# 10XGenomics/supernova

Measured on AMD Instinct MI355X. Metric: Gk-mers/s through count+graph at k=48, 1.2B×150bp; bit-exact counts, higher is better.
Workload: dtype u64

## Files before the change

include/snk.h:

```cpp
#ifndef SNK_H_
#define SNK_H_
#include <stddef.h>
#include <stdint.h>

#ifdef __cplusplus
extern "C" {
#endif

#define SNK_OK 0
#define SNK_E_ARG (-1)
#define SNK_E_HIP (-2)
#define SNK_E_NOGPU (-3)
#define SNK_E_NOMEM (-4)
#define SNK_E_IO (-5)
#define SNK_E_UNSUPPORTED (-6)
#define SNK_E_INTERNAL (-7)

typedef struct snk_ctx snk_ctx;

typedef struct snk_params {
    uint32_t K;
    uint32_t min_qual;
    uint32_t min_freq;
    uint32_t min_bc;
// ... 26 lines not shown
    uint32_t count_tight_slots;
    uint32_t count_screen_ratio_pct;
    uint32_t target_inst;
    uint32_t bucket_fill_pct;
    uint32_t adaptive_buckets;
    uint32_t chunk_kmers;
    uint32_t minimiser_len;
    uint32_t partition_passes;
    uint32_t hot_buckets;
    uint32_t hot_min, hot_factor, hot_class_inst;
    uint32_t exchange_ranges;
    uint32_t join_ranking;
    uint32_t path_lookup;
    uint32_t unitig_bc_cut;
    uint32_t hbv_dev_min, hbv_big;
    uint32_t reserved[9];
    uint32_t last_count_kernel, last_count_limit, last_partition_passes, last_minimiser_len;
} snk_tuning;
void snk_tuning_default(snk_tuning* t);
int snk_ctx_set_tuning(snk_ctx* ctx, const snk_tuning* t, char* err, size_t errcap);
void snk_ctx_get_tuning(const snk_ctx* ctx, snk_tuning* t);
int snk_ctx_set_option(snk_ctx* ctx, const char* name, long long value, char* err, size_t errcap);
int snk_option_check(const char* name, long long value, char* err, size_t errcap);
int snk_ctx_clear_option(snk_ctx* ctx, const char* name);
int snk_ctx_get_option(const snk_ctx* ctx, const char* name, long long* value);
const char* snk_option_name(uint32_t i);
const char* snk_option_doc(uint32_t i);

typedef struct snk_synth_params {
    uint64_t seed;
    uint64_t n_reads;
// ... 416 lines not shown
```

supernova_amd/csrc/snk_count.hip:

```cpp
#include "snk_ctx.h"
#include "snk_common.h"
#include "snk_kernels.h"
#include "snk_stages.h"

namespace {

constexpr uint32_t BC_MULTI = 0xFFFFFFFEu;
constexpr uint32_t BC_IGN = 0xFFFFFFFFu;
static_assert(BC_IGN > BC_MULTI, "barcode states are merged with atomicMax");
#ifndef SNK_TIGHT_TRIES
#define SNK_TIGHT_TRIES 48
#endif
constexpr int MAX_SPLIT_LOG2 = 20;
#define SNK_COUNT_MAXSEG 32
#ifndef SNK_COUNT_THREADS
#define SNK_COUNT_THREADS 768
#endif
#ifndef SNK_SCREEN_ROUNDS
#define SNK_SCREEN_ROUNDS 6
#endif
#ifndef SNK_GSCREEN_SLOTS
#define SNK_GSCREEN_SLOTS 1024
#endif
#ifndef SNK_GSCREEN_BATCH
// ... 10 lines not shown
#endif
#define LDS_LOAD(p) __hip_atomic_load((p), __ATOMIC_RELAXED, __HIP_MEMORY_SCOPE_WORKGROUP)
__device__ __forceinline__ void lds_barrier() { asm volatile("s_waitcnt lgkmcnt(0)\n\ts_barrier" ::: "memory"); }
#ifdef SNK_COUNT_PROF
#define PROF(n) do { if (tid == 0) { const long long _t = clock64(); prof_acc[n] += (unsigned long long)(_t - prof_t); prof_t = _t; } } while (0)
#else
#define PROF(n) do {} while (0)
#endif

__device__ __forceinline__ uint32_t funnel(uint32_t hi, uint32_t lo, uint32_t sh) {
#ifdef SNK_FUNNEL_ALIGNBIT
    return sh ? __builtin_amdgcn_alignbit(hi, lo, 32u - sh) : hi;
#else
    return (uint32_t)(((((uint64_t)hi << 32) | lo) << sh) >> 32);
#endif
}

template <int K> struct lo_t { typedef uint32_t type; };
template <> struct lo_t<60> { typedef uint64_t type; };

template <int K> __device__ __forceinline__ typename lo_t<K>::type lo_pack(uint64_t lo);
template <> __device__ __forceinline__ uint32_t lo_pack<48>(uint64_t lo) { return (uint32_t)(lo >> 32); }
template <> __device__ __forceinline__ uint64_t lo_pack<60>(uint64_t lo) { return lo; }
template <int K> __device__ __forceinline__ uint64_t lo_unpack(typename lo_t<K>::type v);
template <> __device__ __forceinline__ uint64_t lo_unpack<48>(uint32_t v) { return (uint64_t)v << 32; }
template <> __device__ __forceinline__ uint64_t lo_unpack<60>(uint64_t v) { return v; }

template <int K, bool G> struct klo_t { typedef typename lo_t<K>::type type; };
template <int K> struct klo_t<K, true> { typedef uint64_t type; };
template <int K, bool G> __device__ __forceinline__ typename klo_t<K, G>::type klo_pack(uint64_t lo) {
// ... 16 lines not shown
    uint64_t* khi = reinterpret_cast<uint64_t*>(smem_raw);
    lo_type* klo = reinterpret_cast<lo_type*>(khi + SLOTS);
    uint32_t* tag = reinterpret_cast<uint32_t*>(klo + SLOTS);
    uint32_t* cnt = tag + SLOTS;
    uint32_t* bcs = cnt + SLOTS;
    uint32_t* ctxw = bcs + SLOTS;
    uint32_t* rec = ctxw + SLOTS / 4;
    uint32_t* ctl = rec + 8 * BATCH;
    uint32_t* dd = ctl + (TIGHT ? 72 : 64);
    uint32_t* wgt = dd + DD;
    uint16_t* lead = reinterpret_cast<uint16_t*>(wgt + BATCH);
    uint16_t* lpre = lead + BATCH;
    uint16_t* cidx = lpre + BATCH + 2;
    uint32_t* segi = reinterpret_cast<uint32_t*>(smem_raw + (((size_t)(reinterpret_cast<unsigned char*>(cidx + NCI) - smem_raw) + 15) & ~(size_t)15));
    uint16_t* olist = reinterpret_cast<uint16_t*>(segi + 2 * 3 * SNK_COUNT_MAXSEG);
    uint32_t* bcx = reinterpret_cast<uint32_t*>(smem_raw + (((size_t)(reinterpret_cast<unsigned char*>(olist + (TIGHT ? SLOTS - 64 : SLOTS - THREADS - 64)) - smem_raw) + 15) & ~(size_t)15));
    const bool bcset = a.bc_mode > 2;
    constexpr int SROUNDS = (SCREEN && SLOTS <= 1024) ? SNK_GSCREEN_ROUNDS : SNK_SCREEN_ROUNDS;
    static_assert(SROUNDS >= 1 && SROUNDS <= 16, "two cells per register");
    constexpr int SPW = GROUPED ? ((DD + BATCH) / 3 >= 512 ? 512 : 256) : SNK_NGSCREEN_PLANE_WORDS;
    constexpr uint32_t SCB = SPW == 1024 ? 17u : (SPW == 512 ? 18u : 19u);
    constexpr uint32_t SCAND = GROUPED ? (SLOTS <= 1024 ? 2048 : 1024) : 4096;
    uint16_t* cand = reinterpret_cast<uint16_t*>(bcx);
    uint32_t* planes = GROUPED ? dd : reinterpret_cast<uint32_t*>(cand + SCAND);
    static_assert(!SCREEN || (GROUPED && 3 * SPW <= DD + BATCH) || (!GROUPED && K == 48 && SLOTS <= 1024), "no room for the screen's bit planes");
    static_assert(THREADS >= BATCH && THREADS % 64 == 0, "the first BATCH threads own the staged records");
    const int tid = threadIdx.x;
    const int lane = tid & 63;
    const uint32_t LIMIT = TIGHT ? min(a.tight & 0xFFFFu, (uint32_t)SLOTS - 64u) : SLOTS - THREADS - 64;
    const int tight_tries = (int)(a.tight >> 16);
#ifdef SNK_COUNT_PROF
    long long prof_t = clock64();
    unsigned long long prof_acc[8] = {0, 0, 0, 0, 0, 0, 0, 0};
#endif
    auto dma_batch = [&](uint64_t base, uint64_t vend, const uint32_t* bnd, const uint32_t* seg) {
        constexpr int CH = 2 * BATCH;
        uint32_t seg_incl = 0;
        if (MULTI) {
            const uint32_t mylen = (uint32_t)lane < a.nseg ? LDS_LOAD(&seg[2 * SNK_COUNT_MAXSEG + lane]) - LDS_LOAD(&seg[lane]) : 0u;
            seg_incl = snk_wave_scan_incl(mylen);
        }
        constexpr int NR = (CH + THREADS - 1) / THREADS;
        uint32_t gx[NR];
        if (GATHER) {
#pragma unroll
// ... 33 lines not shown
            vend = ((uint64_t)LDS_LOAD(&bnd[3]) << 32) | LDS_LOAD(&bnd[2]);
        }
    };
    const uint32_t G = a.bucket_stride;
    unsigned long long rcur = a.region_cursor[blockIdx.x];
    uint32_t bucket = a.bucket0 + (blockIdx.x + G - a.bucket0 % G) % G;
    uint32_t par = 0;
    {
        uint64_t b0 = 0, e0 = 0;
        if (tid == 0) {
            if (bucket < a.NB) { b0 = a.seg_beg[bucket]; e0 = a.seg_end[bucket]; }
            ctl[4] = (uint32_t)b0; ctl[5] = (uint32_t)(b0 >> 32); ctl[6] = (uint32_t)e0; ctl[7] = (uint32_t)(e0 >> 32);
            ctl[3] = 0;
            ctl[1] = 0; ctl[2] = 0; ctl[8] = 0; ctl[9] = 0; ctl[10] = 0; ctl[11] = 0; ctl[0] = 0;
            if (TIGHT) { ctl[64] = 0; ctl[65] = 0; }
        }
        for (int s = tid; s < SLOTS; s += THREADS) tag[s] = 0;
        if (MULTI && tid < (int)a.nseg) {
            uint64_t b = 0, e = 0;
            if (bucket < a.NB) { b = a.seg_beg[(uint64_t)tid * a.seg_stride + bucket]; e = a.seg_end[(uint64_t)tid * a.seg_stride + bucket]; }
            segi[tid] = (uint32_t)b; segi[SNK_COUNT_MAXSEG + tid] = (uint32_t)(b >> 32); segi[2 * SNK_COUNT_MAXSEG + tid] = (uint32_t)e;
        }
        lds_barrier();
        uint64_t vb, ve;
        bucket_range(ctl + 4, segi, vb, ve);
        dma_batch(vb, ve, ctl + 4, segi);
    }
    bool prefetched = true;
    uint32_t q = 0, bq = 0;
    unsigned long long claims_sum = 0;
    for (; bucket < a.NB; bucket += G) {
    uint32_t sp = 1;
    bool fresh = true;
    uint32_t splits_done = 0;
    const uint32_t nbucket = bucket + G;
    bool seg_pending = true;
    const uint32_t* bcur = ctl + 4 + 8 * par;
    uint32_t* bnext = ctl + 4 + 8 * (par ^ 1u);
    const uint32_t* segc = segi + par * (3 * SNK_COUNT_MAXSEG);
    uint32_t* segn = segi + (par ^ 1u) * (3 * SNK_COUNT_MAXSEG);
    const uint32_t sseg = MULTI ? min((uint32_t)tid, a.nseg - 1u) : 0u;
    auto load_next = [&](uint64_t& nbeg, uint64_t& nend, uint64_t& nsb, uint32_t& nse) {
        nbeg = 0; nend = 0; nsb = 0; nse = 0;
        if (nbucket < a.NB) {
            nbeg = a.seg_beg[nbucket]; nend = a.seg_end[nbucket];
            if (MULTI) { nsb = a.seg_beg[(uint64_t)sseg * a.seg_stride + nbucket]; nse = (uint32_t)a.seg_end[(uint64_t)sseg * a.seg_stride + nbucket]; }
        }
    };
    auto put_down = [&](uint64_t nbeg, uint64_t nend, uint64_t nsb, uint32_t nse) {
        bnext[0] = (uint32_t)nbeg; bnext[1] = (uint32_t)(nbeg >> 32); bnext[2] = (uint32_t)nend; bnext[3] = (uint32_t)(nend >> 32);
        if (MULTI) { segn[sseg] = (uint32_t)nsb; segn[SNK_COUNT_MAXSEG + sseg] = (uint32_t)(nsb >> 32); segn[2 * SNK_COUNT_MAXSEG + sseg] = nse; }
        seg_pending = false;
    };
    uint32_t lg0 = 0, id0 = 0, real_bucket = bucket;
    if (a.vmeta) {
        const uint2 vm = a.vmeta[bucket];
        real_bucket = __builtin_amdgcn_readfirstlane(vm.x);
        lg0 = __builtin_amdgcn_readfirstlane(vm.y >> 24);
        id0 = __builtin_amdgcn_readfirstlane(vm.y & 0xFFFFFFu);
    }
    while (sp) {
// ... 17 lines not shown
            if (seg_pending) {
                uint64_t nbeg, nend, nsb; uint32_t nse;
                load_next(nbeg, nend, nsb, nse);
                put_down(nbeg, nend, nsb, nse);
            }
            lds_barrier();
        }
        PROF(1);
        {
            for (uint64_t base = vbeg; base < vend; base += BATCH) {
                if (!prefetched) dma_batch(base, vend, bcur, segc);
                prefetched = false;
                if (tid < BATCH) wgt[tid] = (SCREEN && GROUPED) ? 0u : 1u;
                if (SCREEN && !GROUPED) { for (int qq = tid; qq < 3 * SPW; qq += THREADS) planes[qq] = 0; }
                for (int q = tid; q < DD; q += THREADS) dd[q] = 0;
                asm volatile("s_waitcnt vmcnt(0)" ::: "memory");
                lds_barrier();
                PROF(2);
                if (tid == 0) { ctl[1 + (q ^ 1u)] = 0; ctl[8 + (q ^ 1u)] = 0; ctl[10 + (bq ^ 1u)] = 0; if (TIGHT) ctl[64 + (q ^ 1u)] = 0; if (SCREEN) ctl[0] = 0; }
                const bool fetch_next = seg_pending;
                uint64_t nbeg = 0, nend = 0, nsb = 0; uint32_t nse = 0;
                if (fetch_next) load_next(nbeg, nend, nsb, nse);
                uint32_t nkm = 0;
                if (tid < BATCH && base + tid < vend) {
                    const uint4 ra = *reinterpret_cast<const uint4*>(rec + 8 * tid), rb = *reinterpret_cast<const uint4*>(rec + 8 * tid + 4);
                    nkm = rb.z & 0x7Fu;
                    if (a.dbg == 5 && ((rb.z >> 7) & 3u) != 3u) nkm = 0;
                    if (!GROUPED && a.dbg != 4 && nkm) {
                        uint32_t h = (ra.x * 0x9E3779B1u) ^ snk_rotl32(ra.y * 0x85EBCA77u, 7) ^ (ra.z * 0xC2B2AE3Du) ^ snk_rotl32(ra.w * 0x27D4EB2Fu, 13)
                                   ^ (rb.x * 0x165667B1u) ^ snk_rotl32(rb.y * 0xcc9e2d51u, 19) ^ (rb.z * 0x1b873593u);
                        h ^= h >> 15; h *= 0x846ca68bu; h ^= h >> 13;
                        uint32_t s = h & (DD - 1);
                        for (;;) {
                            uint32_t v = LDS_LOAD(&dd[s]);
                            if (v == 0) {
                                v = atomicCAS(&dd[s], 0u, (uint32_t)tid + 1u);
                                if (v == 0) break;
                            }
                            const uint32_t L = v - 1u;
                            const uint4 la = *reinterpret_cast<const uint4*>(rec + 8 * L);
                            const uint32_t lb0 = rec[8 * L + 4], lb1 = rec[8 * L + 5], lb2 = rec[8 * L + 6];
                            bool same = ((la.x ^ ra.x) | (la.y ^ ra.y) | (la.z ^ ra.z) | (la.w ^ ra.w) | (lb0 ^ rb.x) | (lb1 ^ rb.y) | (lb2 ^ rb.z)) == 0;
                            if (GROUPED || bcset) same = same && LDS_LOAD(&rec[8 * L + 7]) == rb.w;
                            if (same) {
                                atomicAdd(&wgt[L], 1u);
                                const uint32_t mine = GROUPED ? 0u : rb.w;
                                if (mine >= BC_MULTI) atomicMax(&rec[8 * L + 7], mine);
                                else if (mine) {
                                    uint32_t ob = atomicCAS(&rec[8 * L + 7], 0u, mine);
                                    if (ob != 0 && ob != mine && ob < BC_MULTI) atomicMax(&rec[8 * L + 7], BC_MULTI);
                                }
                                nkm = 0;
                                break;
                            }
                            s = (s + 1) & (DD - 1);
                        }
                    }
                }
                const uint32_t sv = nkm | (nkm ? 0x10000u : 0u);
                uint32_t incl = sv;
                incl = snk_wave_scan_incl(incl);
                uint32_t woff = 0;
                if (lane == 63 && incl) woff = atomicAdd(&ctl[10 + bq], incl);
                woff = __builtin_amdgcn_readlane(woff, 63);
                if (tid < BATCH && nkm) {
                    const uint32_t ex = woff + incl - sv;
                    const uint32_t off = ex & 0xFFFFu, r = ex >> 16;
                    lead[r] = (uint16_t)tid;
                    lpre[r] = (uint16_t)(off + nkm);
                    for (uint32_t w = (off + 31u) >> 5; (w << 5) < off + nkm; ++w) cidx[w] = (uint16_t)r;
// ... 67 lines not shown
                        if (n_iter > SCAND) { screened = false; n_iter = total; }
                    }
                }
                for (uint32_t g0 = 0; g0 < n_iter; g0 += THREADS) {
                    if (TIGHT ? (LDS_LOAD(resv) >> 31) != 0u : LDS_LOAD(occ) > LIMIT) break;
                    uint32_t g = g0 + tid;
                    const bool have = g < n_iter;
                    if (SCREEN && screened && have) g = cand[g];
                    if (have) {
                        uint32_t lr = cidx[g >> 5];
                        uint32_t lend = lpre[lr];
                        while (lend <= g) lend = lpre[++lr];
                        const uint32_t i = lead[lr];
                        const uint32_t* rp = rec + 8 * i;
                        const uint32_t m6 = rp[6], w7 = rp[7];
                        const uint32_t wt = (SCREEN && GROUPED) ? 1u : wgt[i];
                        const uint32_t n_i = m6 & 0x7Fu, hasL = (m6 >> 7) & 1u, hasR = (m6 >> 8) & 1u;
                        const uint32_t j = g + n_i - lend;
                        const uint32_t bst = GROUPED ? 0u : w7;
                        const uint32_t o = hasL + j;
                        const uint32_t wi = o >> 4, sh = (2u * o) & 31u;
                        const uint32_t* wp = rp + wi;
                        const uint32_t P = wp[-1], W0 = wp[0], W1 = wp[1], W2 = wp[2], W3 = wp[3];
                        const uint32_t F0 = funnel(W0, W1, sh), F1 = funnel(W1, W2, sh), F2 = funnel(W2, W3, sh);
                        const uint32_t pb = funnel(P, W0, sh) & 3u;
                        uint32_t F3 = 0, nb;
                        if constexpr (K == 48) nb = (W3 >> (30u - sh)) & 3u;
                        else {
                            static_assert(K == 60, "K is 48 or 60");
                            const uint32_t W4 = wp[4];
                            const uint32_t f3 = funnel(W3, W4, sh);
                            nb = (f3 >> 6) & 3u;
                            F3 = f3 & 0xFFFFFF00u;
// ... 202 lines not shown
                        const uint32_t e = atomicAdd(&a.status[4], 1u);
                        if (e < a.extra_cap) a.extra[e] = make_uint4(real_bucket, (uint32_t)rbase, nvalid | (blockIdx.x << 12), (split_lg << 24) | split_id);
                    }
                }
            }
        }
        claims_sum += nocc;
        if (tid == 0 && nocc > ctl[3]) ctl[3] = nocc;
        q ^= 1u;
        PROF(7);
    }
    if (tid == 0 && splits_done) atomicAdd(&a.status[2], 1u);
    par ^= 1u;
    }
    if (tid == 0) { a.region_cursor[blockIdx.x] = rcur; atomicMax(&a.status[3], ctl[3]); atomicAdd(&a.status[5], (uint32_t)(claims_sum >> 4)); }
    asm volatile("s_waitcnt vmcnt(0)" ::: "memory");
#ifdef SNK_COUNT_PROF
    if (tid == 0) for (int q = 0; q < 8; ++q) atomicAdd(&a.prof[q], prof_acc[q]);
#endif
}

template <int K> struct cfg;
template <> struct cfg<48> { static constexpr int THREADS = SNK_COUNT_THREADS; static constexpr int SLOTS = SNK_COUNT_SLOTS; };
template <> struct cfg<60> { static constexpr int THREADS = SNK_COUNT_THREADS; static constexpr int SLOTS = SNK_COUNT_SLOTS; };

template <int K, bool G>
size_t lds_bytes(uint32_t bc_mode = 0, bool tight = false, bool screen = false) {
    const size_t S = screen ? SNK_GSCREEN_SLOTS : cfg<K>::SLOTS, B = (G && screen && S <= 1024 && K == 48) ? SNK_GSCREEN_BATCH : ((K == 48 && !G && (S >= 2048 || screen)) ? 512 : 256), DD = 2 * B, NCI = B * (K - SNK_M_MIN_OF(K) + 1) / 32 + 2;
    return S * (8 + sizeof(typename klo_t<K, G>::type) + 4 + 4 + 4) + S + 4 * (8 * B + (tight ? 72 : 64) + DD + B) + 2 * (B + B + 2 + NCI) + 16 + 2 * 4 * 3 * SNK_COUNT_MAXSEG + 2 * (tight ? S - 64 : S - cfg<K>::THREADS - 64) + 16 + (bc_mode > 2 ? S * 24 + 16 : 0) + (screen ? (G ? (S <= 1024 ? 4096 : 2048) : 8192 + 3 * SNK_NGSCREEN_PLANE_WORDS * 4) + 16 : 0);
}

template <int K, bool G>
int launch(hipStream_t st, const snk_count_args& a, char* err, size_t errcap) {
    auto kern = a.nseg > 1 ? snk_count_kernel<K, cfg<K>::THREADS, cfg<K>::SLOTS, G, true> : snk_count_kernel<K, cfg<K>::THREADS, cfg<K>::SLOTS, G, false>;
    if (a.gidx) {
        if (a.nseg != 1) return snk_fail(SNK_E_INTERNAL, err, errcap, "count: an index list comes with one segment per bucket");
        kern = snk_count_kernel<K, cfg<K>::THREADS, cfg<K>::SLOTS, G, false, true>;
    }
    const bool tight = a.tight && !a.gidx;
    const bool screen = K == 48 && tight && a.screen >= 2u && a.bc_mode <= 2u;
    static_assert(SNK_GSCREEN_SLOTS <= 1024, "the ungrouped SCREEN instantiation needs the LDS half a table frees");
    if constexpr (K == 48) {
        if (screen) kern = a.nseg > 1 ? snk_count_kernel<K, cfg<K>::THREADS, SNK_GSCREEN_SLOTS, G, true, false, true, true> : snk_count_kernel<K, cfg<K>::THREADS, SNK_GSCREEN_SLOTS, G, false, false, true, true>;
    }
// ... 79 lines not shown
```

supernova_amd/csrc/snk_ctx.h:

```cpp
#pragma once
#include <hip/hip_runtime.h>
#include <stdarg.h>
#include <stdio.h>
#include <string.h>

#include <string>
#include <vector>

#include "../../include/snk.h"
#include "snk_launch.h"
#include "snk_opts.h"
#include "snk_plan.h"

struct snk_ctx {
    int device = 0;
    hipStream_t stream = nullptr;
    hipStream_t cur_stream = nullptr;
    int n_cu = 256;
    size_t lds_per_block = 65536;
    uint64_t device_mem_total = 0;
    double pass_sigma = 0.0;
    uint64_t plan_mapped = 0;
    uint64_t plan_mem = 0;
    struct block { void* p; size_t bytes; bool used; uint64_t serial = 0; uint64_t epoch = 0; };
// ... 18 lines not shown
    size_t cached_bytes = 0;
    uint64_t last_n_kmers = 0, last_n_instances = 0;
    uint64_t last_region_max = 0, last_region_n = 0;
    uint64_t last_bnd = 0, last_bnd_n = 0;
    uint32_t last_ovf = 0, last_ovf_nb = 0;
    uint64_t last_ovf_reads = 0;
    uint64_t last_dense = 0;
    uint32_t count_screen = 0;
    uint32_t count_tight = 0;
    snk_sizing_history sizing;
    uint32_t mlen = 16;
    uint32_t last_extra = 0;
    uint64_t last_input_fp = 0;
    bool have_input_fp = false;
    uint32_t last_count_limit = 0;
    uint32_t last_partition_passes = 1;
    std::vector<unsigned long long> h_region_off;
    snk_opts opts;
    void* shard = nullptr;
    void* host_io = nullptr;
    void (*host_io_free)(void*) = nullptr;
    void* df_io = nullptr;
    void (*df_io_free)(void*) = nullptr;
    void* stream_job = nullptr;
    void (*stream_job_free)(void*) = nullptr;
    void (*stream_job_invalidate)(void*) = nullptr;
    void* shard_host = nullptr;
    void (*shard_host_free)(void*) = nullptr;
};

// ... 25 lines not shown
```

supernova_amd/csrc/snk_opts.hip:

```cpp
#include <stdio.h>
#include <stdlib.h>
#include <string.h>

#include <string>

#include "snk_opts.h"
#ifndef SNK_OPTS_NO_CTX
#include "snk_ctx.h"
#endif

const snk_opt_def snk_opt_defs[SNK_OPT_COUNT] = {
#define X(name, dflt, range, doc) {#name, dflt, range, doc},
    SNK_OPTIONS(X)
#undef X
};

int snk_opt_index(const char* name) {
    if (!name) return -1;
    for (int i = 0; i < SNK_OPT_COUNT; ++i) if (strcmp(snk_opt_defs[i].name, name) == 0) return i;
    return -1;
}
void snk_opts_init(snk_opts* o) { memset(o, 0, sizeof *o); }

int snk_opts_parse(snk_opts* o, const char* text, char* bad, unsigned badcap) {
// ... 135 lines not shown
    long long v;
    for (const tfield& f : tfields) if (get(f.opt, &v)) *reinterpret_cast<uint32_t*>(reinterpret_cast<char*>(t) + f.off) = (uint32_t)v;
    long long tight = 0, ng = 0;
    const bool ts = get(SNK_OPT_count_tight, &tight), ns = get(SNK_OPT_count_screen_ng, &ng);
    if (ns && ng >= 2) t->count_kernel = SNK_COUNT_KERNEL_SCREEN;
    else if (ts && tight) { t->count_kernel = SNK_COUNT_KERNEL_BOOKED; t->count_tight_slots = (uint32_t)tight; }
    else if (ts) t->count_kernel = SNK_COUNT_KERNEL_MARGIN;
    if (get(SNK_OPT_adaptive_buckets, &v)) t->adaptive_buckets = v ? 1 : 2;
    if (get(SNK_OPT_hot, &v)) t->hot_buckets = v ? 1 : 2;
    if (get(SNK_OPT_path_index, &v)) t->path_lookup = v ? 1 : 2;
    if (get(SNK_OPT_join_replicated, &v)) t->join_ranking = v ? 2 : 1;
    t->last_count_limit = ctx->last_count_limit;
    t->last_count_kernel = ctx->count_screen ? SNK_COUNT_KERNEL_SCREEN : (ctx->count_tight ? SNK_COUNT_KERNEL_BOOKED : SNK_COUNT_KERNEL_MARGIN);
    t->last_partition_passes = ctx->last_partition_passes;
    t->last_minimiser_len = ctx->mlen;
}
#endif
```

supernova_amd/csrc/snk_stages.hip:

```cpp
#include <string.h>
#include <cstring>
#include <rocprim/rocprim.hpp>

#include <stdlib.h>
#include <math.h>

#include <cmath>
#include <vector>

#include "snk_ctx.h"
#include "snk_common.h"
#include "snk_graph.h"
#include "snk_kernels.h"
#include "snk_stages.h"


int snk_stage_count_table(snk_ctx* ctx, hipStream_t st, uint32_t K, const void* records, const uint64_t* seg_beg,
                          const uint64_t* seg_end, uint32_t seg_stride, uint32_t nseg, uint32_t NB, uint32_t min_freq, uint32_t bc_mode, uint32_t grouped, uint64_t n_inst_hint,
                          uint32_t* status, bool want_sort, snk_table* out, char* err, size_t errcap, const snk_count_ranges* ranges, snk_count_pilot* pilot,
                          const uint32_t* gidx, bool defer_compact, const snk_hot* hot) {
    if (hot && hot->NBv == 0) hot = nullptr;
    defer_compact = defer_compact && !want_sort && snk_opt_u32(ctx, SNK_OPT_defer_compact) != 0;
    int rc;
    snk_phase_timer tm(st), kt(st);
    tm.mark();
    uint32_t n_regions = 1;
    if ((rc = snk_count_regions(K, grouped, nseg, NB, bc_mode, snk_opt_u32(ctx, SNK_OPT_count_persist), &n_regions, err, errcap))) return rc;
    uint64_t est = n_inst_hint / (min_freq > 1 ? 12 : 1) + 4096;
    const bool tight = ranges && ranges->n > 1 && ranges->replay && min_freq > 1 && ctx->plan_mem && (double)est * 24.0 > 0.10 * (double)ctx->plan_mem;
    if (tight) est = n_inst_hint / 32 + 4096;
    if (ctx->last_n_kmers && ctx->last_n_instances == n_inst_hint) est = ctx->last_n_kmers + ctx->last_n_kmers / (tight ? 8 : 2) + 4096;
    bool range0_probe = tight && !(ctx->last_n_kmers && ctx->last_n_instances == n_inst_hint);
    uint64_t region_cap = est / n_regions + 64;
    if (ctx->last_n_kmers && ctx->last_n_instances == n_inst_hint && ctx->last_region_n == n_regions && ctx->last_region_max + ctx->last_region_max / 4 + 64 > region_cap)
        region_cap = ctx->last_region_max + ctx->last_region_max / 4 + 64;
    snk_u128 *keys_r = nullptr, *keys_a = nullptr, *keys_b = nullptr;
    uint64_t *vals_r = nullptr, *vals_a = nullptr, *vals_b = nullptr;
    unsigned long long *rcur = nullptr, *roff = nullptr;
    uint64_t n_kmers = 0;
    uint32_t h_status[8] = {0, 0, 0, 0, 0, 0, 0, 0};
    {
        void* q;
        if ((rc = snk_ctx_alloc(ctx, (n_regions + 1) * 8ull, &q, err, errcap))) return rc; rcur = (unsigned long long*)q;
        if ((rc = snk_ctx_alloc(ctx, (n_regions + 1) * 8ull, &q, err, errcap))) return rc; roff = (unsigned long long*)q;
    }
    std::vector<unsigned long long> h_rcur(n_regions);
    uint32_t *chunk_n = nullptr, *chunk_base = nullptr;
    uint4* extra = nullptr;
    uint32_t extra_cap = 0;
    if (!want_sort) {
        void* q;
        if ((rc = snk_ctx_alloc(ctx, (NB + 1) * 4ull, &q, err, errcap))) return rc; chunk_n = (uint32_t*)q;
        if ((rc = snk_ctx_alloc(ctx, (NB + 1) * 4ull, &q, err, errcap))) return rc; chunk_base = (uint32_t*)q;
        extra_cap = NB / 8 > (1u << 16) ? NB / 8 : (1u << 16);
        if (ctx->last_extra > extra_cap) extra_cap = ctx->last_extra + ctx->last_extra / 4;
        if (hot) extra_cap += hot->NBv + hot->NBv / 2;
        if (ranges && ranges->hots) extra_cap += NB / 16 + (1u << 16);
    }
    bool pilot_regrown = false;
    for (int attempt = 0; attempt < 4; ++attempt) {
        void* q;
        if (!want_sort) {
            if ((rc = snk_ctx_alloc(ctx, (size_t)extra_cap * 16 + 16, &q, err, errcap))) return rc; extra = (uint4*)q;
            SNK_HIP_TRY(hipMemsetAsync(chunk_n, 0, (NB + 1) * 4ull, st));
        }
        if ((rc = snk_ctx_alloc(ctx, region_cap * n_regions * 16, &q, err, errcap))) return rc; keys_r = (snk_u128*)q;
        if ((rc = snk_ctx_alloc(ctx, region_cap * n_regions * 8, &q, err, errcap))) return rc; vals_r = (uint64_t*)q;
        SNK_HIP_TRY(hipMemsetAsync(rcur, 0, (n_regions + 1) * 8ull, st));
        SNK_HIP_TRY(hipMemsetAsync(status, 0, 32, st));
        snk_count_args ca;
        ca.records = (const uint4*)records;
        ca.seg_beg = seg_beg;
        ca.seg_end = seg_end;
        ca.seg_stride = seg_stride;
        ca.nseg = nseg;
        ca.gidx = gidx;
        ca.vmeta = nullptr;
        ca.NB = NB;
        ca.min_freq = min_freq;
        ca.bc_mode = bc_mode;
        ca.grouped = grouped;
        ca.tight = ctx->count_tight;
        { const uint32_t sc = grouped ? snk_opt_u32(ctx, SNK_OPT_count_screen) : 0u; ca.screen = (sc && min_freq >= (sc >= 2 ? 2u : 3u)) ? std::min(min_freq, 3u) : 0u; }
        if (!grouped && K == 48 && ctx->count_screen && ctx->count_tight && bc_mode <= 2u) ca.screen = std::min(std::min(min_freq, 3u), ctx->count_screen);
// ... 108 lines not shown
            cv.gidx = nullptr;
            cv.vmeta = hot->vmeta;
            cv.NB = hot->NBv;
            cv.bucket0 = 0;
            if ((rc = snk_launch_count(K, st, cv, err, errcap))) return rc;
        }
        if (pilot_regrow) {
            snk_ctx_release_block(ctx, keys_r);
            snk_ctx_release_block(ctx, vals_r);
            if (extra) snk_ctx_release_block(ctx, extra);
            pilot_regrown = true;
            --attempt;
            continue;
        }
        SNK_HIP_TRY(hipMemcpyAsync(h_rcur.data(), rcur, n_regions * 8ull, hipMemcpyDeviceToHost, st));
        SNK_HIP_TRY(hipMemcpyAsync(h_status, status, 32, hipMemcpyDeviceToHost, st));
        SNK_HIP_TRY(snk_sync(st));
#ifdef SNK_COUNT_PROF
        {
            unsigned long long hp[8];
            (void)hipMemcpy(hp, ca.prof, 64, hipMemcpyDeviceToHost);
            unsigned long long tot = 0;
            for (int q = 0; q < 8; ++q) tot += hp[q];
            fprintf(stderr, "[snk prof] count kernel, cycles of thread 0 per phase (%% of total): control %.1f, clear %.1f, stage %.1f, dedupe+scan %.1f, map %.1f, insert %.1f, emit-count %.1f, emit-write %.1f\n",
                    100.0 * hp[0] / tot, 100.0 * hp[1] / tot, 100.0 * hp[2] / tot, 100.0 * hp[3] / tot, 100.0 * hp[4] / tot, 100.0 * hp[5] / tot, 100.0 * hp[6] / tot, 100.0 * hp[7] / tot);
        }
#endif
        if (ca.dbg >= 2) {
            unsigned long long d[3];
            (void)hipMemcpy(d, status + 4, 24, hipMemcpyDeviceToHost);
            fprintf(stderr, "[snk dbg] lane probe iterations %llu, wave-level iterations %llu, max lane iterations in one probe %llu\n", d[0], d[1], d[2]);
        }
        if (h_status[1]) return snk_fail(SNK_E_INTERNAL, err, errcap, h_status[1] == 2 ? "count: a table probe did not terminate" : "count: bucket split depth exceeded");
        unsigned long long mx = 0;
        n_kmers = 0;
        for (uint32_t r = 0; r < n_regions; ++r) { n_kmers += h_rcur[r]; if (h_rcur[r] > mx) mx = h_rcur[r]; }
        const bool extra_ovf = !want_sort && h_status[4] > extra_cap;
        if (!h_status[0] && mx <= region_cap && !extra_ovf) break;
        if (attempt == 3) return snk_fail(SNK_E_INTERNAL, err, errcap, "count: region overflow (%llu > %llu)", mx, (unsigned long long)region_cap);
        snk_ctx_release_block(ctx, keys_r);
        snk_ctx_release_block(ctx, vals_r);
        if (mx > region_cap) region_cap = mx + 64;
        if (extra_ovf) extra_cap = h_status[4] + 64;
// ... 11 lines not shown
        if ((rc = snk_ctx_alloc(ctx, (n_kmers + 1) * 8, &q, err, errcap))) return rc; vals_a = (uint64_t*)q;
        out->keys_r = nullptr; out->vals_r = nullptr; out->region_cap = region_cap;
        if (defer_compact) {
            snk_ctx_release_block(ctx, vals_a);
            vals_a = nullptr;
            out->keys_r = keys_r; out->vals_r = vals_r;
        } else {
            if ((rc = snk_launch_compact_regions(st, keys_r, vals_r, region_cap, n_regions, rcur, roff, keys_a, vals_a, err, errcap))) return rc;
            snk_ctx_release_block(ctx, keys_r);
            snk_ctx_release_block(ctx, vals_r);
        }
    }
    out->buckets_split = h_status[2];
    out->max_slots_used = h_status[3];
    out->distinct = (uint64_t)h_status[5] * 16;
    out->n = n_kmers;
    ctx->last_n_kmers = n_kmers;
    ctx->last_n_instances = n_inst_hint;
    { unsigned long long mxr = 0; for (uint32_t r = 0; r < n_regions; ++r) if (h_rcur[r] > mxr) mxr = h_rcur[r]; ctx->last_region_max = mxr; ctx->last_region_n = n_regions; }
    tm.mark();
    out->sorted = want_sort;
    out->NB = NB;
    out->n_regions = n_regions;
    out->n_extra = want_sort ? 0u : h_status[4];
    if (!want_sort) ctx->last_extra = h_status[4];
    out->chunk_n = chunk_n;
    out->chunk_base = chunk_base;
    out->extra = extra;
    out->region_off = roff;
    if (want_sort) {
// ... 746 lines not shown
```

supernova_amd/lib.py:

```python
from __future__ import annotations

import ctypes as C
from pathlib import Path

import os as _os

_HERE = Path(__file__).resolve().parent
LIB_PATH = Path(_os.environ.get("SNK_LIB_PATH", str(_HERE / "libsnk.so")))


class SnkError(RuntimeError):
    def __init__(self, code: int, msg: str):
        super().__init__(f"libsnk error {code}: {msg}")
        self.code = code


class SnkParams(C.Structure):
    _fields_ = [("K", C.c_uint32), ("min_qual", C.c_uint32), ("min_freq", C.c_uint32), ("min_bc", C.c_uint32),
                ("n_buckets", C.c_uint32), ("flags", C.c_uint32)]


class SnkSynthParams(C.Structure):
    _fields_ = [("seed", C.c_uint64), ("n_reads", C.c_uint64), ("genome_len", C.c_uint64), ("read_len", C.c_uint32),
                ("mol_len", C.c_uint32), ("mols_per_bc", C.c_uint32), ("pairs_per_bc", C.c_uint32),
# ... 73 lines not shown
                ("text_bytes", C.c_uint64), ("token", C.c_uint64)]


class SnkDevIngest(C.Structure):
    _fields_ = [("n_reads", C.c_uint64), ("read_len", C.c_uint32), ("row_words", C.c_uint32), ("qstride", C.c_uint32),
                ("max_len", C.c_uint32), ("rows", C.c_void_p), ("quals", C.c_void_p), ("lens", C.c_void_p), ("bc", C.c_void_p),
                ("text_bytes", C.c_uint64), ("compressed_bytes", C.c_uint64), ("seconds", C.c_double),
                ("decode_wait_seconds", C.c_double), ("n_files", C.c_uint32), ("n_batches", C.c_uint32), ("setup_seconds", C.c_double), ("good_len", C.c_void_p)]


class SnkTuning(C.Structure):
    _fields_ = [("count_kernel", C.c_uint32), ("count_tight_slots", C.c_uint32), ("count_screen_ratio_pct", C.c_uint32), ("target_inst", C.c_uint32),
                ("bucket_fill_pct", C.c_uint32), ("adaptive_buckets", C.c_uint32), ("chunk_kmers", C.c_uint32), ("minimiser_len", C.c_uint32),
                ("partition_passes", C.c_uint32), ("hot_buckets", C.c_uint32), ("hot_min", C.c_uint32), ("hot_factor", C.c_uint32),
                ("hot_class_inst", C.c_uint32), ("exchange_ranges", C.c_uint32), ("join_ranking", C.c_uint32), ("path_lookup", C.c_uint32),
                ("unitig_bc_cut", C.c_uint32), ("hbv_dev_min", C.c_uint32), ("hbv_big", C.c_uint32), ("reserved", C.c_uint32 * 9),
                ("last_count_kernel", C.c_uint32), ("last_count_limit", C.c_uint32), ("last_partition_passes", C.c_uint32),
                ("last_minimiser_len", C.c_uint32)]


class SnkDfInfo(C.Structure):
    _fields_ = [("n_reads", C.c_uint64), ("n_barcodes", C.c_uint64), ("fastb_bytes", C.c_uint64), ("qualp_bytes", C.c_uint64),
                ("bci_bytes", C.c_uint64), ("reserved", C.c_uint64 * 3)]


class SnkShardResult(C.Structure):
    _fields_ = [("rank", C.c_uint32), ("world", C.c_uint32), ("n_reads", C.c_uint64), ("n_instances", C.c_uint64),
                ("n_supermers", C.c_uint64), ("n_buckets_total", C.c_uint64), ("n_kmers", C.c_uint64), ("keys", C.c_void_p),
                ("counts", C.c_void_p), ("ctx", C.c_void_p), ("spectrum", C.c_void_p), ("spectrum_bins", C.c_uint32),
                ("n_circles", C.c_uint32), ("n_unitigs", C.c_uint64), ("unitig_total_bases", C.c_uint64),
                ("unitig_off", C.c_void_p), ("unitig_bases", C.c_void_p), ("unitig_circular", C.c_void_p),
# ... 198 lines not shown
```

Measured before the change: 97.01.

## Fold super-mer records contained in a full record into its per-position weights

Result: slower. 84.95 (-12.4%).

```diff
diff --git a/include/snk.h b/include/snk.h
--- a/include/snk.h
+++ b/include/snk.h
@@ -64,7 +64,8 @@
     uint32_t path_lookup;
     uint32_t unitig_bc_cut;
     uint32_t hbv_dev_min, hbv_big;
-    uint32_t reserved[9];
+    uint32_t reserved[8];
+    uint32_t last_range_folded;
     uint32_t last_count_kernel, last_count_limit, last_partition_passes, last_minimiser_len;
 } snk_tuning;
 void snk_tuning_default(snk_tuning* t);
diff --git a/supernova_amd/csrc/snk_count.hip b/supernova_amd/csrc/snk_count.hip
--- a/supernova_amd/csrc/snk_count.hip
+++ b/supernova_amd/csrc/snk_count.hip
@@ -48,6 +48,21 @@
 #else
     return (uint32_t)(((((uint64_t)hi << 32) | lo) << sh) >> 32);
 #endif
+}
+
+constexpr int SNK_FOLD_KT = 256;
+constexpr uint32_t SNK_FOLD_SUFFIX = 0x5bd1e995u;
+constexpr uint32_t SNK_FOLD_WMASK = 0x3FFu;
+__device__ __forceinline__ uint32_t fold_key_hash(uint32_t a, uint32_t b, uint32_t c, uint32_t d) {
+    uint32_t h = (a * 0x9E3779B1u) ^ snk_rotl32(b * 0x85EBCA77u, 7) ^ (c * 0xC2B2AE3Du) ^ snk_rotl32(d * 0x27D4EB2Fu, 13);
+    h ^= h >> 15; h *= 0x846ca68bu; h ^= h >> 13;
+    return h;
+}
+__device__ __forceinline__ uint32_t fold_key_last(const uint32_t* rp, uint32_t off) {
+    const uint32_t* sp = rp + (off >> 4);
+    const uint32_t sh = 2u * (off & 15u);
+    const uint32_t S0 = sp[0], S1 = sp[1], S2 = sp[2], S3 = sp[3];
+    return fold_key_hash(funnel(S0, S1, sh) ^ SNK_FOLD_SUFFIX, funnel(S1, S2, sh), funnel(S2, S3, sh), (S3 << sh) & 0xC0000000u);
 }
 
 template <int K> struct lo_t { typedef uint32_t type; };
@@ -94,8 +109,12 @@
     uint16_t* cidx = lpre + BATCH + 2;
     uint32_t* segi = reinterpret_cast<uint32_t*>(smem_raw + (((size_t)(reinterpret_cast<unsigned char*>(cidx + NCI) - smem_raw) + 15) & ~(size_t)15));
     uint16_t* olist = reinterpret_cast<uint16_t*>(segi + 2 * 3 * SNK_COUNT_MAXSEG);
-    uint32_t* bcx = reinterpret_cast<uint32_t*>(smem_raw + (((size_t)(reinterpret_cast<unsigned char*>(olist + (TIGHT ? SLOTS - 64 : SLOTS - THREADS - 64)) - smem_raw) + 15) & ~(size_t)15));
+    constexpr bool FOLD = K == 48 && !GROUPED && !SCREEN && !TIGHT;
+    static_assert(!FOLD || (WMAX + K + 1) * 2 <= 192, "a K=48 record keeps its bases in words 0..5");
+    uint32_t* ktab = reinterpret_cast<uint32_t*>(smem_raw + (((size_t)(reinterpret_cast<unsigned char*>(olist + (TIGHT ? SLOTS - 64 : SLOTS - THREADS - 64)) - smem_raw) + 15) & ~(size_t)15));
+    uint32_t* bcx = FOLD ? ktab + SNK_FOLD_KT + 4 : ktab;
     const bool bcset = a.bc_mode > 2;
+    const bool fold_on = FOLD && !bcset && a.dbg != 4 && a.dbg != 6;
     constexpr int SROUNDS = (SCREEN && SLOTS <= 1024) ? SNK_GSCREEN_ROUNDS : SNK_SCREEN_ROUNDS;
     static_assert(SROUNDS >= 1 && SROUNDS <= 16, "two cells per register");
     constexpr int SPW = GROUPED ? ((DD + BATCH) / 3 >= 512 ? 512 : 256) : SNK_NGSCREEN_PLANE_WORDS;
@@ -109,6 +128,14 @@
     const int lane = tid & 63;
     const uint32_t LIMIT = TIGHT ? min(a.tight & 0xFFFFu, (uint32_t)SLOTS - 64u) : SLOTS - THREADS - 64;
     const int tight_tries = (int)(a.tight >> 16);
+    auto kt_put = [&](uint32_t h) {
+        uint32_t ks = h & (SNK_FOLD_KT - 1);
+        const uint32_t ke = (h & ~SNK_FOLD_WMASK) | ((uint32_t)tid + 1u);
+        for (int p = 0; p < 4; ++p) {
+            if (atomicCAS(&ktab[ks], 0u, ke) == 0u) break;
+            ks = (ks + 1) & (SNK_FOLD_KT - 1);
+        }
+    };
 #ifdef SNK_COUNT_PROF
     long long prof_t = clock64();
     unsigned long long prof_acc[8] = {0, 0, 0, 0, 0, 0, 0, 0};
@@ -172,6 +199,7 @@
             ctl[3] = 0;
             ctl[1] = 0; ctl[2] = 0; ctl[8] = 0; ctl[9] = 0; ctl[10] = 0; ctl[11] = 0; ctl[0] = 0;
             if (TIGHT) { ctl[64] = 0; ctl[65] = 0; }
+            if (FOLD) { ktab[SNK_FOLD_KT] = 0; ktab[SNK_FOLD_KT + 1] = 0; }
         }
         for (int s = tid; s < SLOTS; s += THREADS) tag[s] = 0;
         if (MULTI && tid < (int)a.nseg) {
@@ -202,7 +230,11 @@
         nbeg = 0; nend = 0; nsb = 0; nse = 0;
         if (nbucket < a.NB) {
             nbeg = a.seg_beg[nbucket]; nend = a.seg_end[nbucket];
-            if (MULTI) { nsb = a.seg_beg[(uint64_t)sseg * a.seg_stride + nbucket]; nse = (uint32_t)a.seg_end[(uint64_t)sseg * a.seg_stride + nbucket]; }
+            if (MULTI) {
+                uint32_t ss = sseg;
+                if constexpr (FOLD) asm volatile("" : "+v"(ss));
+                nsb = a.seg_beg[(uint64_t)ss * a.seg_stride + nbucket]; nse = (uint32_t)a.seg_end[(uint64_t)ss * a.seg_stride + nbucket];
+            }
         }
     };
     auto put_down = [&](uint64_t nbeg, uint64_t nend, uint64_t nsb, uint32_t nse) {
@@ -250,6 +282,8 @@
                 if (tid < BATCH) wgt[tid] = (SCREEN && GROUPED) ? 0u : 1u;
                 if (SCREEN && !GROUPED) { for (int qq = tid; qq < 3 * SPW; qq += THREADS) planes[qq] = 0; }
                 for (int q = tid; q < DD; q += THREADS) dd[q] = 0;
+                if (FOLD && tid < SNK_FOLD_KT) ktab[tid] = 0;
+                if (FOLD && tid == SNK_FOLD_KT) ktab[SNK_FOLD_KT + 2] = 0;
                 asm volatile("s_waitcnt vmcnt(0)" ::: "memory");
                 lds_barrier();
                 PROF(2);
@@ -257,10 +291,11 @@
                 const bool fetch_next = seg_pending;
                 uint64_t nbeg = 0, nend = 0, nsb = 0; uint32_t nse = 0;
                 if (fetch_next) load_next(nbeg, nend, nsb, nse);
-                uint32_t nkm = 0;
+                uint32_t nkm = 0, rb_z = 0;
                 if (tid < BATCH && base + tid < vend) {
                     const uint4 ra = *reinterpret_cast<const uint4*>(rec + 8 * tid), rb = *reinterpret_cast<const uint4*>(rec + 8 * tid + 4);
                     nkm = rb.z & 0x7Fu;
+                    rb_z = rb.z;
                     if (a.dbg == 5 && ((rb.z >> 7) & 3u) != 3u) nkm = 0;
                     if (!GROUPED && a.dbg != 4 && nkm) {
                         uint32_t h = (ra.x * 0x9E3779B1u) ^ snk_rotl32(ra.y * 0x85EBCA77u, 7) ^ (ra.z * 0xC2B2AE3Du) ^ snk_rotl32(ra.w * 0x27D4EB2Fu, 13)
@@ -271,7 +306,13 @@
                             uint32_t v = LDS_LOAD(&dd[s]);
                             if (v == 0) {
                                 v = atomicCAS(&dd[s], 0u, (uint32_t)tid + 1u);
-                                if (v == 0) break;
+                                if (v == 0) {
+                                    if (FOLD && fold_on && (rb.z & 0x180u) == 0x180u && nkm <= 32u) {
+                                        kt_put(fold_key_hash(ra.x, ra.y, ra.z, ra.w & 0xC0000000u));
+                                        kt_put(fold_key_last(rec + 8 * tid, nkm));
+                                    }
+                                    break;
+                                }
                             }
                             const uint32_t L = v - 1u;
                             const uint4 la = *reinterpret_cast<const uint4*>(rec + 8 * L);
@@ -290,6 +331,71 @@
                                 break;
                             }
                             s = (s + 1) & (DD - 1);
+                        }
+                    }
+                }
+                if (FOLD && fold_on) {
+                    lds_barrier();
+                    PROF(3);
+                    const uint32_t fl = (rb_z >> 7) & 3u;
+                    if (nkm && nkm <= 32u && (fl == 1u || fl == 2u)) {
+                        const bool pre = fl == 1u;
+                        const uint32_t* mp = rec + 8 * tid;
+                        const uint32_t h = pre ? fold_key_hash(mp[0], mp[1], mp[2], mp[3] & 0xC0000000u) : fold_key_last(mp, nkm - 1u);
+                        uint32_t ks = h & (SNK_FOLD_KT - 1);
+                        for (int p = 0; p < 4; ++p) {
+                            const uint32_t e = LDS_LOAD(&ktab[ks]);
+                            if (e == 0) break;
+                            ks = (ks + 1) & (SNK_FOLD_KT - 1);
+                            if ((e ^ h) >> 10) continue;
+                            const uint32_t L = (e & SNK_FOLD_WMASK) - 1u;
+                            const uint32_t nL = rec[8 * L + 6] & 0x7Fu;
+                            if (nkm > nL) continue;
+                            const uint32_t d = pre ? 0u : nL + 1u - nkm;
+                            const uint32_t* lp = rec + 8 * L + (d >> 4);
+                            const uint32_t sd = 2u * (d & 15u);
+                            const uint32_t rbits = 2u * (nkm + (uint32_t)K);
+                            const uint32_t m3 = (uint32_t)(0xFFFFFFFF00000000ull >> min(rbits - 96u, 32u));
+                            const uint32_t m4 = (uint32_t)(0xFFFFFFFF00000000ull >> (rbits > 128u ? rbits - 128u : 0u));
+                            uint32_t diff = funnel(lp[0], lp[1], sd) ^ mp[0];
+                            diff |= funnel(lp[1], lp[2], sd) ^ mp[1];
+                            diff |= funnel(lp[2], lp[3], sd) ^ mp[2];
+                            diff |= (funnel(lp[3], lp[4], sd) & m3) ^ mp[3];
+                            diff |= (funnel(lp[4], lp[5], sd) & m4) ^ mp[4];
+                            if (diff) continue;
+                            const uint32_t w7L = LDS_LOAD(&rec[8 * L + 7]);
+                            if (a.bc_mode == 1u ? w7L == 0u : (a.bc_mode == 2u && w7L < BC_MULTI)) break;
+                            const uint32_t wR = LDS_LOAD(&wgt[tid]);
+                            uint32_t chunk = 0, arr = 0;
+                            for (;;) {
+                                const uint32_t v = LDS_LOAD(&wgt[L]);
+                                if (((v >> 10) & 0xFFFu) + wR > 255u) break;
+                                uint32_t nv = v + (wR << 10);
+                                if ((v >> 22) == 0u) {
+                                    if (!chunk) {
+                                        const uint32_t c = atomicAdd(&ktab[SNK_FOLD_KT + 2], 1u);
+                                        if (c >= (uint32_t)DD / 8u) break;
+                                        *reinterpret_cast<uint4*>(dd + 8 * c) = make_uint4(0u, 0u, 0u, 0u);
+                                        *reinterpret_cast<uint4*>(dd + 8 * c + 4) = make_uint4(0u, 0u, 0u, 0u);
+                                        __builtin_amdgcn_fence(__ATOMIC_RELEASE, "workgroup");
+                                        chunk = c + 1u;
+                                    }
+                                    nv |= chunk << 22;
+                                }
+                                if (atomicCAS(&wgt[L], v, nv) == v) { arr = nv >> 22; break; }
+                            }
+                            if (arr) {
+                                const uint32_t lo = pre ? 0u : nL - nkm, hi = lo + nkm;
+                                uint32_t* wa = dd + 8 * (arr - 1u);
+                                for (uint32_t w = lo >> 2; 4u * w < hi; ++w) {
+                                    const uint32_t b0 = max(lo, 4u * w) - 4u * w, b1 = min(hi, 4u * w + 4u) - 4u * w;
+                                    atomicAdd(&wa[w], ((0x01010101u >> (8u * (4u - b1))) & (0x01010101u << (8u * b0))) * wR);
+                                }
+                                atomicAdd(&ktab[SNK_FOLD_KT], 1u);
+                                atomicAdd(&ktab[SNK_FOLD_KT + 1], nkm);
+                                nkm = 0;
+                            }
+                            break;
                         }
                     }
                 }
@@ -387,9 +493,14 @@
                         const uint32_t i = lead[lr];
                         const uint32_t* rp = rec + 8 * i;
                         const uint32_t m6 = rp[6], w7 = rp[7];
-                        const uint32_t wt = (SCREEN && GROUPED) ? 1u : wgt[i];
+                        uint32_t wt = (SCREEN && GROUPED) ? 1u : wgt[i];
                         const uint32_t n_i = m6 & 0x7Fu, hasL = (m6 >> 7) & 1u, hasR = (m6 >> 8) & 1u;
                         const uint32_t j = g + n_i - lend;
+                        if (FOLD) {
+                            const uint32_t arr = wt >> 22;
+                            wt &= SNK_FOLD_WMASK;
+                            if (arr) wt += (dd[8 * (arr - 1u) + (j >> 2)] >> (8u * (j & 3u))) & 0xFFu;
+                        }
                         const uint32_t bst = GROUPED ? 0u : w7;
                         const uint32_t o = hasL + j;
                         const uint32_t wi = o >> 4, sh = (2u * o) & 31u;
@@ -622,6 +733,10 @@
     par ^= 1u;
     }
     if (tid == 0) { a.region_cursor[blockIdx.x] = rcur; atomicMax(&a.status[3], ctl[3]); atomicAdd(&a.status[5], (uint32_t)(claims_sum >> 4)); }
+    if (FOLD && tid == 0 && ktab[SNK_FOLD_KT]) {
+        atomicAdd(reinterpret_cast<unsigned long long*>(a.status + 6), (unsigned long long)ktab[SNK_FOLD_KT]);
+        atomicAdd(reinterpret_cast<unsigned long long*>(a.status + 8), (unsigned long long)ktab[SNK_FOLD_KT + 1]);
+    }
     asm volatile("s_waitcnt vmcnt(0)" ::: "memory");
 #ifdef SNK_COUNT_PROF
     if (tid == 0) for (int q = 0; q < 8; ++q) atomicAdd(&a.prof[q], prof_acc[q]);
@@ -635,7 +750,7 @@
 template <int K, bool G>
 size_t lds_bytes(uint32_t bc_mode = 0, bool tight = false, bool screen = false) {
     const size_t S = screen ? SNK_GSCREEN_SLOTS : cfg<K>::SLOTS, B = (G && screen && S <= 1024 && K == 48) ? SNK_GSCREEN_BATCH : ((K == 48 && !G && (S >= 2048 || screen)) ? 512 : 256), DD = 2 * B, NCI = B * (K - SNK_M_MIN_OF(K) + 1) / 32 + 2;
-    return S * (8 + sizeof(typename klo_t<K, G>::type) + 4 + 4 + 4) + S + 4 * (8 * B + (tight ? 72 : 64) + DD + B) + 2 * (B + B + 2 + NCI) + 16 + 2 * 4 * 3 * SNK_COUNT_MAXSEG + 2 * (tight ? S - 64 : S - cfg<K>::THREADS - 64) + 16 + (bc_mode > 2 ? S * 24 + 16 : 0) + (screen ? (G ? (S <= 1024 ? 4096 : 2048) : 8192 + 3 * SNK_NGSCREEN_PLANE_WORDS * 4) + 16 : 0);
+    return S * (8 + sizeof(typename klo_t<K, G>::type) + 4 + 4 + 4) + S + 4 * (8 * B + (tight ? 72 : 64) + DD + B) + 2 * (B + B + 2 + NCI) + 16 + 2 * 4 * 3 * SNK_COUNT_MAXSEG + 2 * (tight ? S - 64 : S - cfg<K>::THREADS - 64) + 16 + ((K == 48 && !G && !tight && !screen) ? 4 * (SNK_FOLD_KT + 4) : 0) + (bc_mode > 2 ? S * 24 + 16 : 0) + (screen ? (G ? (S <= 1024 ? 4096 : 2048) : 8192 + 3 * SNK_NGSCREEN_PLANE_WORDS * 4) + 16 : 0);
 }
 
 template <int K, bool G>
diff --git a/supernova_amd/csrc/snk_ctx.h b/supernova_amd/csrc/snk_ctx.h
--- a/supernova_amd/csrc/snk_ctx.h
+++ b/supernova_amd/csrc/snk_ctx.h
@@ -56,6 +56,7 @@
     uint64_t last_input_fp = 0;
     bool have_input_fp = false;
     uint32_t last_count_limit = 0;
+    uint32_t last_range_folded = 0;
     uint32_t last_partition_passes = 1;
     std::vector<unsigned long long> h_region_off;
     snk_opts opts;
diff --git a/supernova_amd/csrc/snk_opts.hip b/supernova_amd/csrc/snk_opts.hip
--- a/supernova_amd/csrc/snk_opts.hip
+++ b/supernova_amd/csrc/snk_opts.hip
@@ -173,5 +173,6 @@
     t->last_count_kernel = ctx->count_screen ? SNK_COUNT_KERNEL_SCREEN : (ctx->count_tight ? SNK_COUNT_KERNEL_BOOKED : SNK_COUNT_KERNEL_MARGIN);
     t->last_partition_passes = ctx->last_partition_passes;
     t->last_minimiser_len = ctx->mlen;
+    t->last_range_folded = ctx->last_range_folded;
 }
 #endif
diff --git a/supernova_amd/csrc/snk_stages.hip b/supernova_amd/csrc/snk_stages.hip
--- a/supernova_amd/csrc/snk_stages.hip
+++ b/supernova_amd/csrc/snk_stages.hip
@@ -38,7 +38,7 @@
     uint64_t *vals_r = nullptr, *vals_a = nullptr, *vals_b = nullptr;
     unsigned long long *rcur = nullptr, *roff = nullptr;
     uint64_t n_kmers = 0;
-    uint32_t h_status[8] = {0, 0, 0, 0, 0, 0, 0, 0};
+    uint32_t h_status[10] = {0, 0, 0, 0, 0, 0, 0, 0, 0, 0};
     {
         void* q;
         if ((rc = snk_ctx_alloc(ctx, (n_regions + 1) * 8ull, &q, err, errcap))) return rc; rcur = (unsigned long long*)q;
@@ -67,7 +67,7 @@
         if ((rc = snk_ctx_alloc(ctx, region_cap * n_regions * 16, &q, err, errcap))) return rc; keys_r = (snk_u128*)q;
         if ((rc = snk_ctx_alloc(ctx, region_cap * n_regions * 8, &q, err, errcap))) return rc; vals_r = (uint64_t*)q;
         SNK_HIP_TRY(hipMemsetAsync(rcur, 0, (n_regions + 1) * 8ull, st));
-        SNK_HIP_TRY(hipMemsetAsync(status, 0, 32, st));
+        SNK_HIP_TRY(hipMemsetAsync(status, 0, 40, st));
         snk_count_args ca;
         ca.records = (const uint4*)records;
         ca.seg_beg = seg_beg;
@@ -206,7 +206,7 @@
             continue;
         }
         SNK_HIP_TRY(hipMemcpyAsync(h_rcur.data(), rcur, n_regions * 8ull, hipMemcpyDeviceToHost, st));
-        SNK_HIP_TRY(hipMemcpyAsync(h_status, status, 32, hipMemcpyDeviceToHost, st));
+        SNK_HIP_TRY(hipMemcpyAsync(h_status, status, 40, hipMemcpyDeviceToHost, st));
         SNK_HIP_TRY(snk_sync(st));
 #ifdef SNK_COUNT_PROF
         {
@@ -218,7 +218,7 @@
                     100.0 * hp[0] / tot, 100.0 * hp[1] / tot, 100.0 * hp[2] / tot, 100.0 * hp[3] / tot, 100.0 * hp[4] / tot, 100.0 * hp[5] / tot, 100.0 * hp[6] / tot, 100.0 * hp[7] / tot);
         }
 #endif
-        if (ca.dbg >= 2) {
+        if (ca.dbg == 2 || ca.dbg == 3) {
             unsigned long long d[3];
             (void)hipMemcpy(d, status + 4, 24, hipMemcpyDeviceToHost);
             fprintf(stderr, "[snk dbg] lane probe iterations %llu, wave-level iterations %llu, max lane iterations in one probe %llu\n", d[0], d[1], d[2]);
@@ -260,6 +260,15 @@
     out->buckets_split = h_status[2];
     out->max_slots_used = h_status[3];
     out->distinct = (uint64_t)h_status[5] * 16;
+    {
+        const uint64_t fr = ((uint64_t)h_status[7] << 32) | h_status[6], fi = ((uint64_t)h_status[9] << 32) | h_status[8];
+        ctx->last_range_folded = fr > 0xFFFFFFFFull ? 0xFFFFFFFFu : (uint32_t)fr;
+#ifdef SNK_COUNT_PROF
+        fprintf(stderr, "[snk prof] count kernel, range fold: %llu records, %llu k-mer instances\n", (unsigned long long)fr, (unsigned long long)fi);
+#else
+        (void)fi;
+#endif
+    }
     out->n = n_kmers;
     ctx->last_n_kmers = n_kmers;
     ctx->last_n_instances = n_inst_hint;
diff --git a/supernova_amd/lib.py b/supernova_amd/lib.py
--- a/supernova_amd/lib.py
+++ b/supernova_amd/lib.py
@@ -111,7 +111,7 @@
                 ("bucket_fill_pct", C.c_uint32), ("adaptive_buckets", C.c_uint32), ("chunk_kmers", C.c_uint32), ("minimiser_len", C.c_uint32),
                 ("partition_passes", C.c_uint32), ("hot_buckets", C.c_uint32), ("hot_min", C.c_uint32), ("hot_factor", C.c_uint32),
                 ("hot_class_inst", C.c_uint32), ("exchange_ranges", C.c_uint32), ("join_ranking", C.c_uint32), ("path_lookup", C.c_uint32),
-                ("unitig_bc_cut", C.c_uint32), ("hbv_dev_min", C.c_uint32), ("hbv_big", C.c_uint32), ("reserved", C.c_uint32 * 9),
+                ("unitig_bc_cut", C.c_uint32), ("hbv_dev_min", C.c_uint32), ("hbv_big", C.c_uint32), ("reserved", C.c_uint32 * 8), ("last_range_folded", C.c_uint32),
                 ("last_count_kernel", C.c_uint32), ("last_count_limit", C.c_uint32), ("last_partition_passes", C.c_uint32),
                 ("last_minimiser_len", C.c_uint32)]
 
```
